# lRomul/sensorium

Hardware: AMD Instinct MI355X
Metric: training clips/sec/GPU (DwiseNeuro fwd+bwd, B=32 T=32 36x64) at 1/2/4/8 GPUs (higher is better)
Workload: dtype bf16

## Files before the change

### sensorium_amd/csrc/dwn_gemm.hip

```cpp
#include "dwn_internal.h"
#include "dwn_launch.h"
#include <type_traits>
int k_zero(void* p, size_t nbytes, hipStream_t s);

#ifndef NN_DMA_NST
#define NN_DMA_NST 3
#endif
#ifndef NN_F32_X3
#define NN_F32_X3 1
#endif

typedef __attribute__((ext_vector_type(8))) short bf16x8_t;
typedef __attribute__((ext_vector_type(4))) short s16x4_t;
typedef __attribute__((ext_vector_type(4))) float f32x4_t;

template <typename T> struct Mma;
template <> struct Mma<bf16_t> {
    static __device__ __forceinline__ void run(const uint4& a, const uint4& b, f32x4_t& acc) {
        acc = __builtin_amdgcn_mfma_f32_16x16x32_bf16(__builtin_bit_cast(bf16x8_t, a),
                                                      __builtin_bit_cast(bf16x8_t, b), acc, 0, 0, 0);
    }
};
template <> struct Mma<float> {
    static __device__ __forceinline__ void run(const uint4& a, const uint4& b, f32x4_t& acc) {
// ... 441 lines not shown
                if (CROWS >= 64 ? (wm == prow0 / 64 || CROWS == 128) : (wm == prow0 / 64)) {
#pragma unroll
                    for (int i = 0; i < 4; ++i) {
                        const int trow = wm * 64 + i * 16 + lr;
                        if (trow >= prow0 && trow < prow0 + CROWS) {
#pragma unroll
                            for (int j = 0; j < NJ; ++j) {
                                const int col = wn * (BN / 2) + j * 16 + lg * 4;
                                unsigned char* dst = sC + sc_off(trow - prow0, col * (int)sizeof(T));
                                if (EPI == EPI_STORE_CAT && n0 + col < g.N) {
                                    const float4 bv = *reinterpret_cast<const float4*>(g.bias + ccol0 + n0 + col);
                                    acc[i][j][0] += bv.x; acc[i][j][1] += bv.y; acc[i][j][2] += bv.z; acc[i][j][3] += bv.w;
                                }
                                if constexpr (TT<T>::IS_BF16) {
                                    uint2 v;
                                    v.x = pk_bf16(acc[i][j][0], acc[i][j][1]);
                                    v.y = pk_bf16(acc[i][j][2], acc[i][j][3]);
                                    *reinterpret_cast<uint2*>(dst) = v;
                                } else {
                                    *reinterpret_cast<float4*>(dst) =
                                        make_float4(acc[i][j][0], acc[i][j][1], acc[i][j][2], acc[i][j][3]);
                                }
                            }
                        }
                    }
                }
                bar();
                if constexpr (fast) {
#pragma unroll
                    for (int it = 0; it < CROWS * CPR / 256; ++it) {
                        const int row = tid / CPR + it * (256 / CPR);
                        const int m = mp + row;
                        const uint4 raw = *reinterpret_cast<const uint4*>(sC + sc_off(row, ch_e * 16));
                        float v[KC];
                        unpack16<T>(raw, v);
                        if constexpr (EPI == EPI_DH3) {
                            float y[KC], dh[KC];
                            unpack16<T>(zraw[it], y);
#pragma unroll
                            for (int i = 0; i < KC; ++i) dh[i] = fmaf(y[i], sc3[i], sh3[i]);
                            silu_grad_n<KC>(dh, dh);
#pragma unroll
                            for (int i = 0; i < KC; ++i) dh[i] = fmaf(v[i], gt3[i], gp3[i]) * dh[i];
                            const uint4 packed = pack16<T>(dh);
                            *reinterpret_cast<uint4*>(Cp + (i64)m * g.ldc + ccol0 + ncol_e) = packed;
                            if (g.stats) {
                                float r[KC];
                                unpack16<T>(packed, r);
#pragma unroll
                                for (int i = 0; i < KC; ++i) { st0[i] += r[i]; st1[i] = fmaf(r[i], y[i], st1[i]); }
                            }
                            continue;
                        }
                        *reinterpret_cast<uint4*>(Cp + (i64)m * g.ldc + ccol0 + ncol_e) = raw;
                        if (g.stats) {
#pragma unroll
                            for (int i = 0; i < KC; ++i) { st0[i] += v[i]; st1[i] += v[i] * v[i]; }
                        }
                        if constexpr (EPI == EPI_DG) {
                            float y[KC];
                            unpack16<T>(zraw[it], y);
#pragma unroll
                            for (int i = 0; i < KC; ++i) dgp[i] += v[i] * y[i];
                        }
                    }
                } else {
#pragma unroll
                for (int it = 0; it < CROWS * CPR / 256; ++it) {
                    const int row = tid / CPR + it * (256 / CPR);
                    const int m = mp + row;
                    if (m >= g.M || ncol >= g.N) continue;
                    const uint4 raw = *reinterpret_cast<const uint4*>(sC + sc_off(row, ch * 16));
                    float v[KC];
                    unpack16<T>(raw, v);
                    if constexpr (EPI == EPI_DH3) {
                        const int b = g.rows_per_sample >= CROWS ? pb3 + (m >= pbound3 ? 1 : 0) : m / g.rows_per_sample;
                        float y[KC], dh[KC];
                        unpack16<T>(zraw[it], y);
                        if (b != gb3) {
                            gb3 = b;
                            ld_coef<KC>(g.gate3 + (i64)b * g.dg_ld + ncol, gt3);
                            ld_coef<KC>(g.dps3 + (i64)b * g.dg_ld + ncol, gp3);
                        }
#pragma unroll
                        for (int i = 0; i < KC; ++i) dh[i] = fmaf(y[i], sc3[i], sh3[i]);
                        silu_grad_n<KC>(dh, dh);
#pragma unroll
                        for (int i = 0; i < KC; ++i) dh[i] = fmaf(v[i], gt3[i], gp3[i]) * dh[i];
                        const uint4 packed = pack16<T>(dh);
                        *reinterpret_cast<uint4*>(Cp + (i64)m * g.ldc + ccol0 + ncol) = packed;
                        if (g.stats) {
                            float r[KC];
                            unpack16<T>(packed, r);
#pragma unroll
                            for (int i = 0; i < KC; ++i) { st0[i] += r[i]; st1[i] = fmaf(r[i], y[i], st1[i]); }
                        }
                        continue;
                    }
                    *reinterpret_cast<uint4*>(Cp + (i64)m * g.ldc + ccol0 + ncol) = raw;
                    if (g.stats) {
#pragma unroll
                        for (int i = 0; i < KC; ++i) { st0[i] += v[i]; st1[i] += v[i] * v[i]; }
                    }
                    if constexpr (EPI == EPI_DG) {
                        const int b = m / g.rows_per_sample;
                        float y[KC];
                        unpack16<T>(zraw[it], y);
                        const int b_pass = mp / g.rows_per_sample;
                        if (b == b_pass) {
#pragma unroll
                            for (int i = 0; i < KC; ++i) dgp[i] += v[i] * y[i];
                        } else {
#pragma unroll
                            for (int i = 0; i < KC; ++i) atomicAdd(g.dg + (i64)b * g.dg_ld + ncol + i, v[i] * y[i]);
                        }
                    }
                }
                }
                if constexpr (EPI == EPI_DG) {
                    const int b_pass = mp / g.rows_per_sample;
                    dg_b = b_pass;
                    const int m_next = mp + CROWS;
                    const bool last = (pass == NPASS - 1) && (mt + 1 == mt_end);
                    const int b_next = (m_next < g.M ? m_next : g.M - 1) / g.rows_per_sample;
                    if (last || b_next != b_pass || m_next >= g.M) flush_dg();
                    else bar();
                } else {
                    bar();
                }
            }
        }
        if constexpr (single && HN) {
            if constexpr (EPI == EPI_READOUT) __syncthreads();
            store_a();
            __syncthreads();
        }
    };
    if constexpr (DMA) {
#pragma unroll
        for (int q = 0; q < NST - 1; ++q) dma_issue();
    }
    else if constexpr (!single) { load_a(mt_beg * BM, 0); load_b(0, mt_beg * BM); }
    for (int mt = mt_beg; mt < mt_end; ++mt) {
        const int m0_ = mt * BM;
        bool fast = m0_ + BM <= g.M;
        if constexpr (EPI == EPI_DG || EPI == EPI_DH3) fast = fast && (m0_ / g.rows_per_sample == (m0_ + BM - 1) / g.rows_per_sample);
        if constexpr (EPI == EPI_READOUT) fast = false;
        using T_ = std::true_type;
        using F_ = std::false_type;
        if constexpr (single) {
            if (mt + 1 < mt_end) { if (fast) tile(mt, T_{}, T_{}); else tile(mt, T_{}, F_{}); }
            else { if (fast) tile(mt, F_{}, T_{}); else tile(mt, F_{}, F_{}); }
        } else if constexpr (DMA) {
            if (fast) tile(mt, F_{}, T_{}); else tile(mt, F_{}, F_{});
        } else {
            tile(mt, F_{}, F_{});
        }
    }
    if constexpr (EPI != EPI_READOUT) {
        if (g.stats) {
            if constexpr (EPI == EPI_DH3) {
                float mu3[KC], is3[KC];
                ld_coef<KC>(g.coef3 + 2 * (i64)g.coef3_ld + ncol_e, mu3);
                ld_coef<KC>(g.coef3 + 3 * (i64)g.coef3_ld + ncol_e, is3);
#pragma unroll
                for (int i = 0; i < KC; ++i) st1[i] = is3[i] * fmaf(-mu3[i], st0[i], st1[i]);
            }
            if (tid < 2 * BN) lred[tid] = 0.f;
            __syncthreads();
            DET_WAVES_BEGIN
            if (ncol < g.N) {
#pragma unroll
                for (int i = 0; i < KC; ++i) {
                    atomicAdd(&lred[ch * KC + i], st0[i]);
                    atomicAdd(&lred[BN + ch * KC + i], st1[i]);
                }
            }
            DET_WAVES_END
            __syncthreads();
            DET_ENTER();
            if (tid < 2 * BN) {
                int col = tid % BN, which = tid / BN;
                if (n0 + col < g.N)
                    stat_add(g.stats, (int)(blockIdx.x % DWN_NREP), g.stat_nchan, which, ccol0 + n0 + col, lred[tid]);
            }
        }
    }
    DET_EXIT();
}

template <typename T, int ALD, int EPI, int BNv, int SINGLE>
static int launch_nn_k(const GemmNN& g, hipStream_t s) {
    const int BM = 128;
    const int ntm = (g.M + BM - 1) / BM;
    const int ntn = (g.N + BNv - 1) / BNv;
    const int bpc = resident_bpc(gemm_nn_kernel<T, ALD, EPI, BNv, SINGLE>, 256, 0, 1);
    int nranges = (256 * bpc) / (ntn * g.groups);
    if (nranges > ntm) nranges = ntm;
    if (nranges < 1) nranges = 1;
    while (nranges > 1 && (nranges * ntn) % 8 != 0) --nranges;
    if ((nranges * ntn) % 8 != 0) nranges = 8;
    dim3 grid(nranges * ntn, g.groups);
    if constexpr (!TT<T>::IS_BF16 && NN_F32_X3 != 0) {
        if (g.f32_split != 0) {
            hipLaunchKernelGGL((gemm_nn_kernel<T, ALD, EPI, BNv, SINGLE, true>), grid, dim3(256), 0, s, g);
            DWN_CHECK_LAUNCH();
            return 0;
        }
    }
    hipLaunchKernelGGL((gemm_nn_kernel<T, ALD, EPI, BNv, SINGLE>), grid, dim3(256), 0, s, g);
    DWN_CHECK_LAUNCH();
    return 0;
}

template <int ALD, int EPI> struct HasSingle {
    static constexpr bool value = (ALD == LD_PLAIN && (EPI == EPI_STORE || EPI == EPI_DG || EPI == EPI_DH3)) || (ALD == LD_PE && EPI == EPI_STORE);
};
template <int ALD, int EPI> struct HasSingle2 {
    static constexpr bool value = ALD == LD_PLAIN && (EPI == EPI_STORE || EPI == EPI_DG || EPI == EPI_DH3);
};

static bool nn_use_dma(const GemmNN& g, int bn) {
    if (g.K % 64 != 0 || g.K < 128 || (g.epi == EPI_STORE_CAT && g.K1 % 64 != 0)) return false;
    if (g.epi == EPI_READOUT) return false;
    if (g.b_sample_stride) return true;
    const long long tiles = (long long)((g.M + 127) / 128) * ((g.N + bn - 1) / bn) * g.groups;
    return tiles <= 5 * 256 && g.K >= 512;
}

template <typename T, int ALD, int EPI>
static int launch_nn_t(const GemmNN& g, hipStream_t s) {
    constexpr int BK = 128 / (int)sizeof(T);
    const bool n64 = g.N <= 64 || (EPI == EPI_DH3 && !(TT<T>::IS_BF16 && g.N % 128 == 0));
    if constexpr (HasSingle<ALD, EPI>::value) {
        if (g.K <= BK) return n64 ? launch_nn_k<T, ALD, EPI, 64, 1>(g, s) : launch_nn_k<T, ALD, EPI, 128, 1>(g, s);
    }
    if constexpr (HasSingle2<ALD, EPI>::value) {
        if (g.K <= 2 * BK && !g.b_sample_stride)
            return n64 ? launch_nn_k<T, ALD, EPI, 64, 2>(g, s) : launch_nn_k<T, ALD, EPI, 128, 2>(g, s);
    }
    if constexpr (ALD == LD_PLAIN && TT<T>::IS_BF16) {
        if (nn_use_dma(g, n64 ? 64 : 128))
            return n64 ? launch_nn_k<T, ALD, EPI, 64, 3>(g, s) : launch_nn_k<T, ALD, EPI, 128, 3>(g, s);
    }
    return n64 ? launch_nn_k<T, ALD, EPI, 64, 0>(g, s) : launch_nn_k<T, ALD, EPI, 128, 0>(g, s);
}

template <typename T>
static int launch_nn_d(const GemmNN& g, hipStream_t s) {
    if (g.K % TT<T>::KC != 0) return dwn_set_error(-2, "gemm_nn: K must be a multiple of the 16-byte vector");
    if (g.epi == EPI_READOUT) {
        if (g.a_kind == LD_BNACT) return launch_nn_t<T, LD_BNACT, EPI_READOUT>(g, s);
        if (g.a_kind == LD_PLAIN) return launch_nn_t<T, LD_PLAIN, EPI_READOUT>(g, s);
        return dwn_set_error(-3, "gemm_nn: unsupported loader for readout epilogue");
    }
    if (g.N % TT<T>::KC != 0) return dwn_set_error(-2, "gemm_nn: N must be a multiple of the 16-byte vector");
    if (g.epi == EPI_DG) {
        if (g.s3 || g.t3) return dwn_set_error(-3, "gemm_nn: the dg epilogue reads the activated z3; s3/t3 must be NULL");
        if (g.a_kind == LD_PLAIN && g.groups == 1) return launch_nn_t<T, LD_PLAIN, EPI_DG>(g, s);
        return dwn_set_error(-3, "gemm_nn: unsupported loader for dg epilogue");
    }
    if (g.epi == EPI_DH3) {
        if (g.a_kind != LD_PLAIN || g.groups != 1 || !g.y3 || !g.gate3 || !g.dps3 || !g.coef3 || g.rows_per_sample <= 0)
            return dwn_set_error(-3, "gemm_nn: the dh3 epilogue needs a plain loader, groups == 1, y3, gate3, dps3, coef3, rows_per_sample");
        return launch_nn_t<T, LD_PLAIN, EPI_DH3>(g, s);
    }
    if (g.epi == EPI_STORE_CAT) {
        if (g.a_kind != LD_PLAIN || g.groups != 1 || g.K1 <= 0 || g.K1 % TT<T>::KC || !g.a2 || !g.bias)
            return dwn_set_error(-3, "gemm_nn: K-concat epilogue needs a plain loader, groups == 1, a2, bias and K1 % vector == 0");
        return launch_nn_t<T, LD_PLAIN, EPI_STORE_CAT>(g, s);
    }
    switch (g.a_kind) {
        case LD_PLAIN: return launch_nn_t<T, LD_PLAIN, EPI_STORE>(g, s);
        case LD_PE: return launch_nn_t<T, LD_PE, EPI_STORE>(g, s);
        case LD_BNACT: return launch_nn_t<T, LD_BNACT, EPI_STORE>(g, s);
        case LD_AFFINE2: return launch_nn_t<T, LD_AFFINE2, EPI_STORE>(g, s);
        case LD_GATE: return launch_nn_t<T, LD_GATE, EPI_STORE>(g, s);
    }
    return dwn_set_error(-3, "gemm_nn: unsupported loader kind");
}

int launch_gemm_nn(const GemmNN& g, int dtype, hipStream_t s) {
    if (g.M <= 0 || g.N <= 0 || g.K <= 0) return 0;
    if (g.b_sample_stride) {
        const int bk = dtype == DWN_BF16 ? 64 : 32;
        if (g.b_rows_per_sample <= 0 || g.b_rows_per_sample % 128 || g.groups != 1 || g.K <= bk)
            return dwn_set_error(-2, "gemm_nn: per-sample weights need b_rows_per_sample % 128 == 0, groups == 1, K > one k-tile");
    }
    if (gemm_nn_kd_eligible(g, dtype)) return launch_gemm_nn_kd(g, s);
    if (gemm_nn_xl_eligible(g, dtype)) return launch_gemm_nn_xl(g, s);
    return dtype == DWN_BF16 ? launch_nn_d<bf16_t>(g, s) : launch_nn_d<float>(g, s);
}

#ifndef TN_MINW_PLAIN
#define TN_MINW_PLAIN 3
#endif
template <typename T> static __device__ __forceinline__ uint4 ones_vec();
template <> __device__ __forceinline__ uint4 ones_vec<bf16_t>() { return make_uint4(0x3F803F80u, 0x3F803F80u, 0x3F803F80u, 0x3F803F80u); }
template <> __device__ __forceinline__ uint4 ones_vec<float>() { return make_uint4(0x3F800000u, 0x3F800000u, 0x3F800000u, 0x3F800000u); }
template <typename T> struct TnCfg;
template <> struct TnCfg<bf16_t> { static constexpr int PAD = 32; };
template <> struct TnCfg<float>  { static constexpr int PAD = 64; };

template <int PLD, int QLD> struct TnOcc {
    static constexpr int value = (PLD == LD_AFFINE2 || PLD == LD_DY3 || QLD == LD_AFFINE2 || QLD == LD_DY3) ? 2 : TN_MINW_PLAIN;
};
template <typename T, int PLD, int QLD>
__global__ __launch_bounds__(256, (TnOcc<PLD, QLD>::value)) void gemm_tn_kernel(const GemmTN g) {
    constexpr int KC = TT<T>::KC;
    constexpr int BR = 128, BC = 128, BMK = TT<T>::IS_BF16 ? 64 : 32;
    constexpr int RS = BR * (int)sizeof(T) + TnCfg<T>::PAD;
    constexpr int CPR = BR / KC;
    constexpr int NCH = BMK * CPR / 256;
    __shared__ __attribute__((aligned(16))) unsigned char smem[2 * BMK * RS];
    unsigned char* sP = smem;
    unsigned char* sQ = smem + BMK * RS;

    const int tid = threadIdx.x;
    const int ntc = (g.Cc + BC - 1) / BC;
    int tile_id = blockIdx.x, split_id = blockIdx.y;
    {
        const unsigned total = gridDim.x * gridDim.y, bid = blockIdx.x + gridDim.x * blockIdx.y;
        if ((total & 7u) == 0u) {
            const unsigned lid = (bid & 7u) * (total >> 3) + (bid >> 3);
            tile_id = (int)(lid % gridDim.x);
            split_id = (int)(lid / gridDim.x);
        }
    }
    const int rt = tile_id / ntc, ct = tile_id % ntc;
    const int r0 = rt * BR, c0 = ct * BC;
    const int grp = blockIdx.z;
    const int Rl = g.R_load > 0 ? g.R_load : g.R;
    const int pcol0 = grp * Rl, qcol0 = grp * g.Cc;
    i64 mbeg = (i64)split_id * g.rows_per_split;
    i64 mend = mbeg + g.rows_per_split;
    if (mend > g.M) mend = g.M;
    i64 dw_off = 0;
    if (g.rows_per_sample > 0) {
        const int b = split_id / g.splits_per_sample, j = split_id % g.splits_per_sample;
        mbeg = (i64)b * g.rows_per_sample + (i64)j * g.rows_per_split;
        mend = mbeg + g.rows_per_split;
        const i64 send = (i64)(b + 1) * g.rows_per_sample;
        if (mend > send) mend = send;
        dw_off = (i64)b * g.dw_sample_stride;
    }

    const int wave = tid >> 6, lane = tid & 63;
    const int wm = wave >> 1, wn = wave & 1;
    const int lr = lane & 15, lg = lane >> 4;

    f32x4_t acc[4][4];
#pragma unroll
    for (int i = 0; i < 4; ++i)
#pragma unroll
        for (int j = 0; j < 4; ++j) acc[i][j] = f32x4_t{0.f, 0.f, 0.f, 0.f};

    uint4 p1[NCH], p2[NCH], q1[NCH], q2[NCH];
    i64 ld_mb = 0;
    const int chq = tid % CPR;
    const int rcol = r0 + chq * KC, ccol = c0 + chq * KC;
    const bool rok = rcol < Rl, cok = ccol < g.Cc;
    ColCoef<(PLD == LD_PE || PLD == LD_CAT1) ? LD_PLAIN : PLD, T> cfp;
    ColCoef<QLD == LD_PE ? LD_PLAIN : QLD, T> cfq;
    if (rok) cfp.load(g.p, pcol0 + rcol);
    if (cok) cfq.load(g.q, qcol0 + ccol);
    const T* Pp = reinterpret_cast<const T*>(g.p.p);
    const T* Pq = reinterpret_cast<const T*>(g.p.q);
    const T* Qp = reinterpret_cast<const T*>(g.q.p);
    const T* Qq = reinterpret_cast<const T*>(g.q.q);
    i64 pld = g.p.ld;
    int pcol = pcol0 + rcol;
    [[maybe_unused]] bool p_ones = false;
    if constexpr (PLD == LD_CAT1) {
        if (rcol >= g.p.cat_c1 + g.p.cat_c2) p_ones = true;
        else if (rcol >= g.p.cat_c1) { Pp = Pq; pld = g.p.ld2; pcol = rcol - g.p.cat_c1; }
    }
    auto load_tiles = [&](i64 mb) {
        ld_mb = mb;
#pragma unroll
        for (int i = 0; i < NCH; ++i) {
            i64 m = mb + tid / CPR + (256 / CPR) * i;
            const bool mok = m < mend;
            i64 offp = (mok && rok) ? m * pld + pcol : 0;
            if constexpr (PLD == LD_CAT1) { if (p_ones) offp = 0; }
            const i64 offq = (mok && cok) ? m * g.q.ld + qcol0 + ccol : 0;
            if constexpr (PLD != LD_PE) {
                p1[i] = *reinterpret_cast<const uint4*>(Pp + offp);
                if constexpr (decltype(cfp)::two_tensors) p2[i] = *reinterpret_cast<const uint4*>(Pq + offp);
            } else {
                p1[i] = (mok && rok) ? load_op_packed<LD_PE, T>(g.p, m, pcol0 + rcol) : make_uint4(0, 0, 0, 0);
            }
            if constexpr (QLD != LD_PE) {
                q1[i] = *reinterpret_cast<const uint4*>(Qp + offq);
                if constexpr (decltype(cfq)::two_tensors) q2[i] = *reinterpret_cast<const uint4*>(Qq + offq);
            } else {
                q1[i] = (mok && cok) ? load_op_packed<LD_PE, T>(g.q, m, qcol0 + ccol) : make_uint4(0, 0, 0, 0);
            }
        }
    };
    auto store_tiles = [&]() {
        const uint4 z4 = make_uint4(0, 0, 0, 0);
#pragma unroll
        for (int i = 0; i < NCH; ++i) {
            int mrow = tid / CPR + (256 / CPR) * i;
            const i64 m = ld_mb + mrow;
            const bool mok = m < mend;
            uint4 vp, vq;
            if constexpr (PLD == LD_PE) vp = p1[i];
            else if constexpr (PLD == LD_CAT1) vp = !(mok && rok) ? z4 : p_ones ? ones_vec<T>() : p1[i];
            else if constexpr (decltype(cfp)::two_tensors) vp = (mok && rok) ? cfp.apply(g.p, (unsigned)m, p1[i], p2[i]) : z4;
            else vp = (mok && rok) ? cfp.apply(g.p, (unsigned)m, p1[i], z4) : z4;
            if constexpr (QLD == LD_PE) vq = q1[i];
            else if constexpr (decltype(cfq)::two_tensors) vq = (mok && cok) ? cfq.apply(g.q, (unsigned)m, q1[i], q2[i]) : z4;
            else vq = (mok && cok) ? cfq.apply(g.q, (unsigned)m, q1[i], z4) : z4;
            *reinterpret_cast<uint4*>(sP + mrow * RS + chq * 16) = vp;
            *reinterpret_cast<uint4*>(sQ + mrow * RS + chq * 16) = vq;
        }
    };

    if (mbeg < mend) {
        load_tiles(mbeg);
        store_tiles();
    }
    __syncthreads();
    for (i64 mb = mbeg; mb < mend; mb += BMK) {
        const bool has_next = (mb + BMK) < mend;
        if (has_next) load_tiles(mb + BMK);
        if constexpr (TT<T>::IS_BF16) {
            const int q = lr >> 2, p = lr & 3;
#pragma unroll
            for (int kb = 0; kb < BMK / 32; ++kb) {
                bf16x8_t af[4], bfr[4];
                const int rb = kb * 32 + 8 * lg + q;
#pragma unroll
                for (int i = 0; i < 4; ++i) {
                    int colb = (wm * 64 + i * 16 + 4 * p) * 2;
                    auto lo = __builtin_amdgcn_ds_read_tr16_b64_v4i16(
                        (__attribute__((address_space(3))) s16x4_t*)(sP + rb * RS + colb));
                    auto hi = __builtin_amdgcn_ds_read_tr16_b64_v4i16(
                        (__attribute__((address_space(3))) s16x4_t*)(sP + (rb + 4) * RS + colb));
                    af[i] = bf16x8_t{lo[0], lo[1], lo[2], lo[3], hi[0], hi[1], hi[2], hi[3]};
                }
#pragma unroll
                for (int j = 0; j < 4; ++j) {
                    int colb = (wn * 64 + j * 16 + 4 * p) * 2;
                    auto lo = __builtin_amdgcn_ds_read_tr16_b64_v4i16(
                        (__attribute__((address_space(3))) s16x4_t*)(sQ + rb * RS + colb));
                    auto hi = __builtin_amdgcn_ds_read_tr16_b64_v4i16(
                        (__attribute__((address_space(3))) s16x4_t*)(sQ + (rb + 4) * RS + colb));
                    bfr[j] = bf16x8_t{lo[0], lo[1], lo[2], lo[3], hi[0], hi[1], hi[2], hi[3]};
                }
#pragma unroll
                for (int i = 0; i < 4; ++i)
#pragma unroll
                    for (int j = 0; j < 4; ++j)
                        acc[i][j] = __builtin_amdgcn_mfma_f32_16x16x32_bf16(af[i], bfr[j], acc[i][j], 0, 0, 0);
            }
        } else {
#pragma unroll
            for (int ks = 0; ks < BMK / 4; ++ks) {
                float af[4], bfr[4];
#pragma unroll
                for (int i = 0; i < 4; ++i)
                    af[i] = *reinterpret_cast<const float*>(sP + (ks * 4 + lg) * RS + (wm * 64 + i * 16 + lr) * 4);
#pragma unroll
                for (int j = 0; j < 4; ++j)
                    bfr[j] = *reinterpret_cast<const float*>(sQ + (ks * 4 + lg) * RS + (wn * 64 + j * 16 + lr) * 4);
#pragma unroll
                for (int i = 0; i < 4; ++i)
#pragma unroll
                    for (int j = 0; j < 4; ++j)
                        acc[i][j] = __builtin_amdgcn_mfma_f32_16x16x4f32(af[i], bfr[j], acc[i][j], 0, 0, 0);
            }
        }
        __syncthreads();
        if (has_next) {
            store_tiles();
            __syncthreads();
        }
    }
    if (mbeg >= mend) { DET_EXIT(); return; }
    DET_ENTER();
    float* dw = g.dw + (i64)grp * g.R * g.lddw + dw_off;
#pragma unroll
    for (int i = 0; i < 4; ++i)
#pragma unroll
        for (int j = 0; j < 4; ++j)
#pragma unroll
            for (int r = 0; r < 4; ++r) {
                int rr = r0 + wm * 64 + i * 16 + lg * 4 + r;
                int cc = c0 + wn * 64 + j * 16 + lr;
                if (rr < g.R && cc < g.Cc) {
                    if (g.overwrite == 2) dw[(i64)rr * g.lddw + cc] = acc[i][j][r];
                    else if (g.dw_f64) atomicAdd(reinterpret_cast<double*>(g.dw) + (i64)grp * g.R * g.lddw + dw_off + (i64)rr * g.lddw + cc, (double)acc[i][j][r]);
                    else atomicAdd(dw + (i64)rr * g.lddw + cc, acc[i][j][r]);
                }
            }
    DET_EXIT();
}

#define TRY_(x) do { int rc__ = (x); if (rc__ != 0) return rc__; } while (0)
#ifndef TN_SLOTS
#define TN_SLOTS 2
#endif
#ifndef TN_F64_SLOTS
#define TN_F64_SLOTS 2
#endif
template <typename T, int PLD, int QLD>
static int launch_tn_t(const GemmTN& g_in, hipStream_t s) {
    GemmTN g = g_in;
    if (g.rows_per_sample > 0) {
        if (g.groups != 1 || g.M % g.rows_per_sample) return dwn_set_error(-2, "gemm_tn: per-sample mode needs groups == 1 and M % rows_per_sample == 0");
        int bpc = resident_bpc(gemm_tn_kernel<T, PLD, QLD>, 256, 0, 1);
        const int nb = g.M / g.rows_per_sample;
        const int tiles = ((g.R + 127) / 128) * ((g.Cc + 127) / 128);
        if (bpc > TN_SLOTS) bpc = TN_SLOTS;
        int J = (256 * bpc) / (tiles * nb);
        const int maxj = (g.rows_per_sample + 511) / 512;
        if (J > maxj) J = maxj;
        if (J < 1) J = 1;
        int rows = (g.rows_per_sample + J - 1) / J;
        rows = (rows + 63) / 64 * 64;
        g.rows_per_split = rows;
        g.splits_per_sample = (g.rows_per_sample + rows - 1) / rows;
        g.nsplit = nb * g.splits_per_sample;
    } else if (g.nsplit <= 0) {
        int bpc = resident_bpc(gemm_tn_kernel<T, PLD, QLD>, 256, 0, 1);
        if (bpc > TN_SLOTS) bpc = TN_SLOTS;
        if (g.dw_f64 && bpc > TN_F64_SLOTS) bpc = TN_F64_SLOTS;
        const int tiles = ((g.R + 127) / 128) * ((g.Cc + 127) / 128) * g.groups;
        int want = (256 * bpc) / tiles;
        const int maxsplit = (int)((g.M + 511) / 512);
        if (want > maxsplit) want = maxsplit;
        if (want < 1) want = 1;
        const int tiles_g = ((g.R + 127) / 128) * ((g.Cc + 127) / 128);
        for (int w = want; w >= 1 && w > want - 8; --w) {
            i64 rows = (g.M + w - 1) / w;
            rows = (rows + 63) / 64 * 64;
            g.rows_per_split = (int)rows;
            g.nsplit = (int)((g.M + rows - 1) / rows);
            if (((tiles_g * g.nsplit) & 7) == 0) break;
        }
        if (((tiles_g * g.nsplit) & 7) != 0) {
            i64 rows = (g.M + want - 1) / want;
            rows = (rows + 63) / 64 * 64;
            g.rows_per_split = (int)rows;
            g.nsplit = (int)((g.M + rows - 1) / rows);
        }
    }
    if (g.dw_f64 && (g.overwrite || g.rows_per_sample > 0)) return dwn_set_error(-2, "gemm_tn: dw_f64 excludes overwrite and per-sample mode");
    if (g.overwrite) {
        if (g.rows_per_sample > 0 || g.lddw != g.Cc) return dwn_set_error(-2, "gemm_tn: overwrite needs lddw == Cc and no per-sample mode");
        if (g.nsplit == 1) g.overwrite = 2;
        else TRY_(k_zero(g.dw, (size_t)g.groups * g.R * g.lddw * sizeof(float), s));
    }
    dim3 grid(((g.R + 127) / 128) * ((g.Cc + 127) / 128), g.nsplit, g.groups);
    hipLaunchKernelGGL((gemm_tn_kernel<T, PLD, QLD>), grid, dim3(256), 0, s, g);
    DWN_CHECK_LAUNCH();
    return 0;
}

template <typename T>
static int launch_tn_d(const GemmTN& g, hipStream_t s) {
    const int Rl = g.R_load > 0 ? g.R_load : g.R;
    if (Rl % TT<T>::KC != 0 || g.Cc % TT<T>::KC != 0)
        return dwn_set_error(-2, "gemm_tn: R and Cc must be multiples of the 16-byte vector");
    const int pk = g.p_kind, qk = g.q_kind;
    if (pk == LD_AFFINE2 && qk == LD_PE) return launch_tn_t<T, LD_AFFINE2, LD_PE>(g, s);
    if (pk == LD_PLAIN && qk == LD_BNACT) return launch_tn_t<T, LD_PLAIN, LD_BNACT>(g, s);
    if (pk == LD_PLAIN && qk == LD_GATE) return launch_tn_t<T, LD_PLAIN, LD_GATE>(g, s);
    if (pk == LD_PLAIN && qk == LD_PLAIN) return launch_tn_t<T, LD_PLAIN, LD_PLAIN>(g, s);
    if (pk == LD_AFFINE2 && qk == LD_PLAIN) return launch_tn_t<T, LD_AFFINE2, LD_PLAIN>(g, s);
    if (pk == LD_CAT1 && qk == LD_PLAIN) {
        if (g.p.cat_c1 <= 0 || g.p.cat_c2 < 0 || g.p.cat_c1 % TT<T>::KC || g.p.cat_c2 % TT<T>::KC || g.groups != 1 ||
            g.R < g.p.cat_c1 + g.p.cat_c2 || (g.p.cat_c2 > 0 && !g.p.q))
            return dwn_set_error(-2, "gemm_tn: LD_CAT1 needs groups == 1, segment widths in 16-byte vectors and R >= cat_c1 + cat_c2");
        return launch_tn_t<T, LD_CAT1, LD_PLAIN>(g, s);
    }
    return dwn_set_error(-3, "gemm_tn: unsupported loader combination");
}

int launch_gemm_tn(const GemmTN& g_in, int dtype, hipStream_t s) {
    if (g_in.M <= 0 || g_in.R <= 0 || g_in.Cc <= 0) return 0;
    const GemmTN& g = g_in;
    return dtype == DWN_BF16 ? launch_tn_d<bf16_t>(g, s) : launch_tn_d<float>(g, s);
}

static __device__ __forceinline__ unsigned pwb_pack2(float a, float b) { return pk_bf16(a, b); }
namespace pwb {
constexpr int CIN = 64, BM = 128;
constexpr int RS = 160;
template <int NKC> struct Cfg {
    static constexpr int E = NKC * 64, KCAT = E + CIN;
    static constexpr int WRS = KCAT * 2 + 16;
    static constexpr int SW_BYTES = CIN * WRS, SD_BYTES = BM * RS, SX_BYTES = BM * RS;
    static constexpr int MAP_INTS = 512;
    static constexpr int LDS_BYTES = SW_BYTES + 2 * SD_BYTES + 2 * SX_BYTES + 7 * CIN * 4 + MAP_INTS * 4;
};
}
struct PwbGather { const int* hinv; const int* winv; int Hin, Win, Hout, Wout; };
template <int NKC>
__global__ __launch_bounds__(512) __attribute__((amdgpu_waves_per_eu(2, 2))) void pw_bwd_fused_kernel(const bf16_t* __restrict__ dh1, const bf16_t* __restrict__ a0,
                                                       const bf16_t* __restrict__ bp, const float* __restrict__ r3,
                                                       bf16_t* __restrict__ da0, float* __restrict__ tacc, int M,
                                                       const bf16_t* __restrict__ res, const float* __restrict__ res_coef, int res_n,
                                                       const PwbGather gq) {
    using namespace pwb;
    constexpr int E = Cfg<NKC>::E, KCAT = Cfg<NKC>::KCAT, WRS = Cfg<NKC>::WRS;
    constexpr int SW_BYTES = Cfg<NKC>::SW_BYTES, SD_BYTES = Cfg<NKC>::SD_BYTES, SX_BYTES = Cfg<NKC>::SX_BYTES;
    extern __shared__ __attribute__((aligned(16))) unsigned char pwb_smem[];
    unsigned char* const smem = pwb_smem;
    unsigned char* sW = smem;
    unsigned char* sD = smem + SW_BYTES;
    unsigned char* sX = sD + 2 * SD_BYTES;
    float* sR3 = reinterpret_cast<float*>(sX + 2 * SX_BYTES);
    const int tid = threadIdx.x, wave = tid >> 6, lane = tid & 63;
    const int lr = lane & 15, lg = lane >> 4;
    const int wm = wave & 3, wn = wave >> 2;
    if (tid < CIN) sR3[tid] = r3[tid];
    const bool gather = res && gq.hinv;
    if (res) for (int i = tid; i < (gather ? 3 : 1) * res_n * CIN; i += 512) sR3[CIN + i] = res_coef[i];
    int* sMap = reinterpret_cast<int*>(sR3 + 7 * CIN);
    if (gather) for (int i = tid; i < gq.Hin + gq.Win; i += 512) sMap[i] = i < gq.Hin ? gq.hinv[i] : gq.winv[i - gq.Hin];
    const RasterIdx ridx(gather ? gq.Hin : 1, gather ? gq.Win : 1);
    for (int c = tid; c < CIN * (KCAT / 8); c += 512) {
        const int n = c / (KCAT / 8), kc8 = c % (KCAT / 8);
        *reinterpret_cast<uint4*>(sW + n * WRS + kc8 * 16) = *reinterpret_cast<const uint4*>(bp + (size_t)n * KCAT + kc8 * 8);
    }
    f32x4_t acc_dw[NKC][2], acc_ga[2], acc_s[2];
#pragma unroll
    for (int k = 0; k < NKC; ++k) { acc_dw[k][0] = f32x4_t{0, 0, 0, 0}; acc_dw[k][1] = f32x4_t{0, 0, 0, 0}; }
    acc_ga[0] = acc_ga[1] = acc_s[0] = acc_s[1] = f32x4_t{0, 0, 0, 0};
    const int ntiles = M / BM;
    const int ch = tid & 7;
    const int row_a = tid >> 3;
    struct Pair { uint4 lo, hi; };
    Pair rd[NKC], rx;
    auto fetch_a0 = [&](int tile) {
        const bf16_t* src = a0 + ((size_t)tile * BM + row_a) * CIN + ch * 8;
        return Pair{*reinterpret_cast<const uint4*>(src), *reinterpret_cast<const uint4*>(src + (size_t)64 * CIN)};
    };
    auto fetch_chunk = [&](int tile, int kc) {
        const bf16_t* src = dh1 + ((size_t)tile * BM + row_a) * E + kc * 64 + ch * 8;
        return Pair{*reinterpret_cast<const uint4*>(src), *reinterpret_cast<const uint4*>(src + (size_t)64 * E)};
    };
    int tile = blockIdx.x;
    {
        const int t0 = tile < ntiles ? tile : 0;
        rx = fetch_a0(t0);
#pragma unroll
        for (int kc = 0; kc < NKC; ++kc) rd[kc] = fetch_chunk(t0, kc);
    }
    __syncthreads();
    const int q = lr >> 2, p = lr & 3;
    const bf16x8_t ones = {(short)0x3F80, (short)0x3F80, (short)0x3F80, (short)0x3F80, (short)0x3F80, (short)0x3F80, (short)0x3F80, (short)0x3F80};
    int tpar = 0, step = 0;
    for (; tile < ntiles; tile += gridDim.x, tpar ^= 1) {
        const size_t m0 = (size_t)tile * BM;
        const int ntile = tile + (int)gridDim.x < ntiles ? tile + (int)gridDim.x : tile;
        unsigned char* sXt = sX + tpar * SX_BYTES;
        *reinterpret_cast<uint4*>(sXt + row_a * RS + ch * 16) = rx.lo;
        *reinterpret_cast<uint4*>(sXt + (row_a + 64) * RS + ch * 16) = rx.hi;
        rx = fetch_a0(ntile);
        f32x4_t acc_da[2][2];
        uint2 rres[2][2][2];
        bool rgat[2] = {true, true};
#pragma unroll
        for (int i = 0; i < 2; ++i) { acc_da[i][0] = f32x4_t{0, 0, 0, 0}; acc_da[i][1] = f32x4_t{0, 0, 0, 0}; }
#pragma unroll
        for (int kc = 0; kc < NKC; ++kc) {
            unsigned char* sDk = sD + ((step + kc) & 1) * SD_BYTES;
            *reinterpret_cast<uint4*>(sDk + row_a * RS + ch * 16) = rd[kc].lo;
            *reinterpret_cast<uint4*>(sDk + (row_a + 64) * RS + ch * 16) = rd[kc].hi;
            nn_lds_barrier();
            rd[kc] = fetch_chunk(ntile, kc);
            if (kc == NKC - 3 && res) {
#pragma unroll
                for (int i = 0; i < 2; ++i) {
                    size_t rrow = m0 + wm * 32 + i * 16 + lr;
                    if (gather) {
                        unsigned bt; int hi, wi;
                        ridx.decode((unsigned)rrow, bt, hi, wi);
                        const int ho = sMap[hi], wo = sMap[gq.Hin + wi];
                        rgat[i] = ho >= 0 && wo >= 0;
                        rrow = rgat[i] ? ((size_t)bt * gq.Hout + ho) * gq.Wout + wo : 0;
                    }
#pragma unroll
                    for (int j = 0; j < 2; ++j) {
                        const bf16_t* rp_ = res + rrow * (size_t)(res_n * CIN) + wn * 32 + j * 16 + 4 * lg;
                        rres[i][j][0] = *reinterpret_cast<const uint2*>(rp_);
                        rres[i][j][1] = *reinterpret_cast<const uint2*>(rp_ + (res_n > 1 ? CIN : 0));
                    }
                }
            }
#pragma unroll
            for (int kb = 0; kb < 2; ++kb) {
                bf16x8_t af[2], wf[2];
#pragma unroll
                for (int i = 0; i < 2; ++i)
                    af[i] = *reinterpret_cast<const bf16x8_t*>(sDk + (wm * 32 + i * 16 + lr) * RS + (kb * 4 + lg) * 16);
#pragma unroll
                for (int j = 0; j < 2; ++j)
                    wf[j] = *reinterpret_cast<const bf16x8_t*>(sW + (wn * 32 + j * 16 + lr) * WRS + (kc * 64 + kb * 32 + lg * 8) * 2);
#pragma unroll
                for (int i = 0; i < 2; ++i)
#pragma unroll
                    for (int j = 0; j < 2; ++j)
                        acc_da[i][j] = __builtin_amdgcn_mfma_f32_16x16x32_bf16(wf[j], af[i], acc_da[i][j], 0, 0, 0);
            }
#pragma unroll
            for (int kb = 0; kb < BM / 32; ++kb) {
                const int rb = kb * 32 + 8 * lg + q;
                bf16x8_t ef, cf[2];
                {
                    const int colb = (wm * 16 + 4 * p) * 2;
                    auto lo = __builtin_amdgcn_ds_read_tr16_b64_v4i16((__attribute__((address_space(3))) s16x4_t*)(sDk + rb * RS + colb));
                    auto hi = __builtin_amdgcn_ds_read_tr16_b64_v4i16((__attribute__((address_space(3))) s16x4_t*)(sDk + (rb + 4) * RS + colb));
                    ef = bf16x8_t{lo[0], lo[1], lo[2], lo[3], hi[0], hi[1], hi[2], hi[3]};
                }
#pragma unroll
                for (int j = 0; j < 2; ++j) {
                    const int colb = (wn * 32 + j * 16 + 4 * p) * 2;
                    auto lo = __builtin_amdgcn_ds_read_tr16_b64_v4i16((__attribute__((address_space(3))) s16x4_t*)(sXt + rb * RS + colb));
                    auto hi = __builtin_amdgcn_ds_read_tr16_b64_v4i16((__attribute__((address_space(3))) s16x4_t*)(sXt + (rb + 4) * RS + colb));
                    cf[j] = bf16x8_t{lo[0], lo[1], lo[2], lo[3], hi[0], hi[1], hi[2], hi[3]};
                }
#pragma unroll
                for (int j = 0; j < 2; ++j)
                    acc_dw[kc][j] = __builtin_amdgcn_mfma_f32_16x16x32_bf16(ef, cf[j], acc_dw[kc][j], 0, 0, 0);
            }
            if (kc == 0) {
#pragma unroll
                for (int kb = 0; kb < 2; ++kb) {
                    bf16x8_t af[2], wf[2];
#pragma unroll
                    for (int i = 0; i < 2; ++i)
                        af[i] = *reinterpret_cast<const bf16x8_t*>(sXt + (wm * 32 + i * 16 + lr) * RS + (kb * 4 + lg) * 16);
#pragma unroll
                    for (int j = 0; j < 2; ++j)
                        wf[j] = *reinterpret_cast<const bf16x8_t*>(sW + (wn * 32 + j * 16 + lr) * WRS + (E + kb * 32 + lg * 8) * 2);
#pragma unroll
                    for (int i = 0; i < 2; ++i)
#pragma unroll
                        for (int j = 0; j < 2; ++j)
                            acc_da[i][j] = __builtin_amdgcn_mfma_f32_16x16x32_bf16(wf[j], af[i], acc_da[i][j], 0, 0, 0);
                }
#pragma unroll
                for (int kb = 0; kb < BM / 32; ++kb) {
                    const int rb = kb * 32 + 8 * lg + q;
                    bf16x8_t ef, cf[2];
                    {
                        const int colb = (wm * 16 + 4 * p) * 2;
                        auto lo = __builtin_amdgcn_ds_read_tr16_b64_v4i16((__attribute__((address_space(3))) s16x4_t*)(sXt + rb * RS + colb));
                        auto hi = __builtin_amdgcn_ds_read_tr16_b64_v4i16((__attribute__((address_space(3))) s16x4_t*)(sXt + (rb + 4) * RS + colb));
                        ef = bf16x8_t{lo[0], lo[1], lo[2], lo[3], hi[0], hi[1], hi[2], hi[3]};
                    }
#pragma unroll
                    for (int j = 0; j < 2; ++j) {
                        const int colb = (wn * 32 + j * 16 + 4 * p) * 2;
                        auto lo = __builtin_amdgcn_ds_read_tr16_b64_v4i16((__attribute__((address_space(3))) s16x4_t*)(sXt + rb * RS + colb));
                        auto hi = __builtin_amdgcn_ds_read_tr16_b64_v4i16((__attribute__((address_space(3))) s16x4_t*)(sXt + (rb + 4) * RS + colb));
                        cf[j] = bf16x8_t{lo[0], lo[1], lo[2], lo[3], hi[0], hi[1], hi[2], hi[3]};
                    }
#pragma unroll
                    for (int j = 0; j < 2; ++j) {
                        acc_ga[j] = __builtin_amdgcn_mfma_f32_16x16x32_bf16(ef, cf[j], acc_ga[j], 0, 0, 0);
                        if (wm == 0) acc_s[j] = __builtin_amdgcn_mfma_f32_16x16x32_bf16(ones, cf[j], acc_s[j], 0, 0, 0);
                    }
                }
            }
        }
        step += NKC;
#pragma unroll
        for (int i = 0; i < 2; ++i)
#pragma unroll
            for (int j = 0; j < 2; ++j) {
                const size_t m = m0 + wm * 32 + i * 16 + lr;
                const int n = wn * 32 + j * 16 + 4 * lg;
                const float4 b4 = *reinterpret_cast<const float4*>(sR3 + n);
                float o[4] = {acc_da[i][j][0] + b4.x, acc_da[i][j][1] + b4.y, acc_da[i][j][2] + b4.z, acc_da[i][j][3] + b4.w};
                if (res) {
                    const int rc = res_n * CIN;
                    float x4[4] = {0.f, 0.f, 0.f, 0.f};
                    if (gather) {
                        const uint2 xv = *reinterpret_cast<const uint2*>(sXt + (wm * 32 + i * 16 + lr) * RS + n * 2);
                        x4[0] = __uint_as_float(xv.x << 16); x4[1] = __uint_as_float(xv.x & 0xffff0000u);
                        x4[2] = __uint_as_float(xv.y << 16); x4[3] = __uint_as_float(xv.y & 0xffff0000u);
                    }
#pragma unroll
                    for (int jj = 0; jj < 2; ++jj) {
                        if (jj >= res_n || !rgat[i]) break;
                        const uint2 rv = rres[i][j][jj];
                        const float4 c4 = *reinterpret_cast<const float4*>(sR3 + CIN + jj * CIN + n);
                        float t[4] = {c4.x * __uint_as_float(rv.x << 16), c4.y * __uint_as_float(rv.x & 0xffff0000u),
                                      c4.z * __uint_as_float(rv.y << 16), c4.w * __uint_as_float(rv.y & 0xffff0000u)};
                        if (gather) {
                            const float4 a2 = *reinterpret_cast<const float4*>(sR3 + CIN + rc + jj * CIN + n);
                            const float4 a3 = *reinterpret_cast<const float4*>(sR3 + CIN + 2 * rc + jj * CIN + n);
                            t[0] += fmaf(a2.x, x4[0], a3.x); t[1] += fmaf(a2.y, x4[1], a3.y);
                            t[2] += fmaf(a2.z, x4[2], a3.z); t[3] += fmaf(a2.w, x4[3], a3.w);
                        }
                        o[0] += t[0]; o[1] += t[1]; o[2] += t[2]; o[3] += t[3];
                    }
                }
                uint2 v = make_uint2(pwb_pack2(o[0], o[1]), pwb_pack2(o[2], o[3]));
                *reinterpret_cast<uint2*>(da0 + m * CIN + n) = v;
            }
    }
    DET_ENTER();
#pragma unroll
    for (int kc = 0; kc < NKC; ++kc)
#pragma unroll
        for (int j = 0; j < 2; ++j)
#pragma unroll
            for (int r = 0; r < 4; ++r)
                atomicAdd(tacc + (size_t)(kc * 64 + wm * 16 + 4 * lg + r) * CIN + wn * 32 + j * 16 + lr, acc_dw[kc][j][r]);
#pragma unroll
    for (int j = 0; j < 2; ++j) {
#pragma unroll
        for (int r = 0; r < 4; ++r)
            atomicAdd(tacc + (size_t)(E + wm * 16 + 4 * lg + r) * CIN + wn * 32 + j * 16 + lr, acc_ga[j][r]);
        if (wm == 0 && lg == 0) atomicAdd(tacc + (size_t)KCAT * CIN + wn * 32 + j * 16 + lr, acc_s[j][0]);
    }
    DET_EXIT();
}


bool pw_bwd_fused_supported(int dtype, long long M, int E, int Cin) {
    return dtype == DWN_BF16 && (E == 448 || E == 384) && Cin == pwb::CIN && M > 0 && M % pwb::BM == 0 && M <= 0x7fffffffLL;
}
template <int NKC>
static int launch_pw_bwd_fused_t(const void* dh1, const void* a0, const void* bp, const float* r3, void* da0, float* tacc,
                                 long long M, const void* res, const float* res_coef, int res_n, const PwbGather& gq, hipStream_t s) {
    auto kern = pw_bwd_fused_kernel<NKC>;
    {
        hipError_t e = lds_opt_in(kern, pwb::Cfg<NKC>::LDS_BYTES);
        if (e != hipSuccess) return dwn_set_error((int)e, hipGetErrorString(e));
    }
    int grid = 256;
    if (grid > (int)(M / pwb::BM)) grid = (int)(M / pwb::BM);
    hipLaunchKernelGGL(kern, dim3(grid), dim3(512), pwb::Cfg<NKC>::LDS_BYTES, s, (const bf16_t*)dh1, (const bf16_t*)a0,
                       (const bf16_t*)bp, r3, (bf16_t*)da0, tacc, (int)M, (const bf16_t*)res, res_coef, res_n, gq);
    DWN_CHECK_LAUNCH();
    return 0;
}
int launch_pw_bwd_fused(const void* dh1, const void* a0, const void* bp, const float* r3, void* da0, float* tacc,
                        long long M, int E, int Cin, int dtype, const void* res, const float* res_coef, int res_n,
                        const int* hinv, const int* winv, int Hin, int Win, int Hout, int Wout, hipStream_t s) {
    PwbGather gq; gq.hinv = hinv; gq.winv = winv; gq.Hin = Hin; gq.Win = Win; gq.Hout = Hout; gq.Wout = Wout;
    if (res && hinv && (!winv || Hin <= 0 || Win <= 0 || Hout <= 0 || Wout <= 0 || M % ((long long)Hin * Win) || Hin + Win > 512))
        return dwn_set_error(-2, "pw_bwd_fused: the gathered shortcut form needs both inverse maps, M = frames * Hin * Win and Hin + Win <= 512");
    if (!pw_bwd_fused_supported(dtype, M, E, Cin))
        return dwn_set_error(-3, "pw_bwd_fused: built for bf16, Cin = 64, E = 448 or 384, M % 128 == 0 only");
    if (res && (!res_coef || res_n < 1 || res_n > 2)) return dwn_set_error(-3, "pw_bwd_fused: the residual term needs res_coef and res_n in {1, 2}");
    return E == 448 ? launch_pw_bwd_fused_t<7>(dh1, a0, bp, r3, da0, tacc, M, res, res_coef, res_n, gq, s)
                    : launch_pw_bwd_fused_t<6>(dh1, a0, bp, r3, da0, tacc, M, res, res_coef, res_n, gq, s);
}
```

Measured before the change: 1475.

## Add register-ring prefetch with double-buffered LDS and fold ones-row bias into TN GEMM

For plain and concat-with-ones weight-gradient GEMMs, the kernel now keeps a register ring of prefetched global tiles and ping-pongs two LDS buffers, so each k-step needs one barrier instead of two. For the concat-with-ones case it accumulates column sums of Q in registers and writes them to the bias rows from the last real row tile. This removes the extra 128-row tile that existed only to hold the ones row. The cost is more registers and twice the shared memory, with occupancy capped at 2 for these variants. Ablation macros and an optional LDS-staged flush are also added but are off by default.

```diff
diff --git a/sensorium_amd/csrc/dwn_gemm.hip b/sensorium_amd/csrc/dwn_gemm.hip
--- a/sensorium_amd/csrc/dwn_gemm.hip
+++ b/sensorium_amd/csrc/dwn_gemm.hip
@@ -767,17 +767,35 @@
 template <> struct TnCfg<bf16_t> { static constexpr int PAD = 32; };
 template <> struct TnCfg<float>  { static constexpr int PAD = 64; };
 
+#ifndef TN_RING
+#define TN_RING 2
+#endif
+#ifndef TN_FLUSH_LDS
+#define TN_FLUSH_LDS 0
+#endif
+#ifndef TN_ONES_FOLD
+#define TN_ONES_FOLD 1
+#endif
+template <int PLD, int QLD> struct TnRing {
+    static constexpr int value = ((PLD == LD_PLAIN || PLD == LD_CAT1) && QLD == LD_PLAIN) ? TN_RING : 0;
+};
 template <int PLD, int QLD> struct TnOcc {
-    static constexpr int value = (PLD == LD_AFFINE2 || PLD == LD_DY3 || QLD == LD_AFFINE2 || QLD == LD_DY3) ? 2 : TN_MINW_PLAIN;
+    static constexpr int value = (TnRing<PLD, QLD>::value > 0 || PLD == LD_AFFINE2 || PLD == LD_DY3 || QLD == LD_AFFINE2 || QLD == LD_DY3)
+                                     ? 2 : TN_MINW_PLAIN;
 };
+#if defined(TN_ABL_LOADONLY) && !defined(TN_ABL_NOFLUSH)
+#define TN_ABL_NOFLUSH
+#endif
 template <typename T, int PLD, int QLD>
-__global__ __launch_bounds__(256, (TnOcc<PLD, QLD>::value)) void gemm_tn_kernel(const GemmTN g) {
+__global__ __launch_bounds__(256, (TnOcc<PLD, QLD>::value)) void gemm_tn_kernel(const GemmTN g, const int ones_rt, const int ones_n) {
     constexpr int KC = TT<T>::KC;
     constexpr int BR = 128, BC = 128, BMK = TT<T>::IS_BF16 ? 64 : 32;
     constexpr int RS = BR * (int)sizeof(T) + TnCfg<T>::PAD;
     constexpr int CPR = BR / KC;
     constexpr int NCH = BMK * CPR / 256;
-    __shared__ __attribute__((aligned(16))) unsigned char smem[2 * BMK * RS];
+    constexpr int RING = TnRing<PLD, QLD>::value;
+    constexpr int TILE = 2 * BMK * RS;
+    __shared__ __attribute__((aligned(16))) unsigned char smem[(RING > 0 ? 2 : 1) * TILE];
     unsigned char* sP = smem;
     unsigned char* sQ = smem + BMK * RS;
 
@@ -878,11 +896,157 @@
             if constexpr (QLD == LD_PE) vq = q1[i];
             else if constexpr (decltype(cfq)::two_tensors) vq = (mok && cok) ? cfq.apply(g.q, (unsigned)m, q1[i], q2[i]) : z4;
             else vq = (mok && cok) ? cfq.apply(g.q, (unsigned)m, q1[i], z4) : z4;
+#ifdef TN_ABL_LOADONLY
+            asm volatile("" :: "v"(vp.x), "v"(vp.y), "v"(vp.z), "v"(vp.w), "v"(vq.x), "v"(vq.y), "v"(vq.z), "v"(vq.w));
+#else
             *reinterpret_cast<uint4*>(sP + mrow * RS + chq * 16) = vp;
             *reinterpret_cast<uint4*>(sQ + mrow * RS + chq * 16) = vq;
+#endif
         }
     };
 
+    auto mma_tile = [&](const unsigned char* tP, const unsigned char* tQ) __attribute__((always_inline)) {
+#ifdef TN_ABL_LOADONLY
+        (void)tP; (void)tQ;
+#else
+        if constexpr (TT<T>::IS_BF16) {
+            const int q = lr >> 2, p = lr & 3;
+#pragma unroll
+            for (int kb = 0; kb < BMK / 32; ++kb) {
+                bf16x8_t af[4], bfr[4];
+                const int rb = kb * 32 + 8 * lg + q;
+#pragma unroll
+                for (int i = 0; i < 4; ++i) {
+                    int colb = (wm * 64 + i * 16 + 4 * p) * 2;
+                    auto lo = __builtin_amdgcn_ds_read_tr16_b64_v4i16(
+                        (__attribute__((address_space(3))) s16x4_t*)(tP + rb * RS + colb));
+                    auto hi = __builtin_amdgcn_ds_read_tr16_b64_v4i16(
+                        (__attribute__((address_space(3))) s16x4_t*)(tP + (rb + 4) * RS + colb));
+                    af[i] = bf16x8_t{lo[0], lo[1], lo[2], lo[3], hi[0], hi[1], hi[2], hi[3]};
+                }
+#pragma unroll
+                for (int j = 0; j < 4; ++j) {
+                    int colb = (wn * 64 + j * 16 + 4 * p) * 2;
+                    auto lo = __builtin_amdgcn_ds_read_tr16_b64_v4i16(
+                        (__attribute__((address_space(3))) s16x4_t*)(tQ + rb * RS + colb));
+                    auto hi = __builtin_amdgcn_ds_read_tr16_b64_v4i16(
+                        (__attribute__((address_space(3))) s16x4_t*)(tQ + (rb + 4) * RS + colb));
+                    bfr[j] = bf16x8_t{lo[0], lo[1], lo[2], lo[3], hi[0], hi[1], hi[2], hi[3]};
+                }
+#pragma unroll
+                for (int i = 0; i < 4; ++i)
+#pragma unroll
+                    for (int j = 0; j < 4; ++j)
+                        acc[i][j] = __builtin_amdgcn_mfma_f32_16x16x32_bf16(af[i], bfr[j], acc[i][j], 0, 0, 0);
+            }
+        } else {
+#pragma unroll
+            for (int ks = 0; ks < BMK / 4; ++ks) {
+                float af[4], bfr[4];
+#pragma unroll
+                for (int i = 0; i < 4; ++i)
+                    af[i] = *reinterpret_cast<const float*>(tP + (ks * 4 + lg) * RS + (wm * 64 + i * 16 + lr) * 4);
+#pragma unroll
+                for (int j = 0; j < 4; ++j)
+                    bfr[j] = *reinterpret_cast<const float*>(tQ + (ks * 4 + lg) * RS + (wn * 64 + j * 16 + lr) * 4);
+#pragma unroll
+                for (int i = 0; i < 4; ++i)
+#pragma unroll
+                    for (int j = 0; j < 4; ++j)
+                        acc[i][j] = __builtin_amdgcn_mfma_f32_16x16x4f32(af[i], bfr[j], acc[i][j], 0, 0, 0);
+            }
+        }
+#endif
+    };
+    if constexpr (RING > 0) {
+        constexpr int U = (RING % 2 == 0) ? RING : 2 * RING;
+        uint4 rp[RING][NCH], rq[RING][NCH];
+        [[maybe_unused]] const bool sum_q = PLD == LD_CAT1 && rt == ones_rt;
+        [[maybe_unused]] f32x4_t cs0 = {0.f, 0.f, 0.f, 0.f}, cs1 = {0.f, 0.f, 0.f, 0.f};
+        auto ring_load = [&](uint4 (&dp)[NCH], uint4 (&dq)[NCH], i64 mb) __attribute__((always_inline)) {
+#pragma unroll
+            for (int i = 0; i < NCH; ++i) {
+                const i64 m = mb + tid / CPR + (256 / CPR) * i;
+                const bool mok = m < mend;
+                i64 offp = (mok && rok) ? m * pld + pcol : 0;
+                if constexpr (PLD == LD_CAT1) { if (p_ones) offp = 0; }
+                const i64 offq = (mok && cok) ? m * g.q.ld + qcol0 + ccol : 0;
+                dp[i] = *reinterpret_cast<const uint4*>(Pp + offp);
+                dq[i] = *reinterpret_cast<const uint4*>(Qp + offq);
+            }
+        };
+        auto ring_store = [&](const uint4 (&dp)[NCH], const uint4 (&dq)[NCH], i64 mb, int buf) __attribute__((always_inline)) {
+#pragma unroll
+            for (int i = 0; i < NCH; ++i) {
+                const int mrow = tid / CPR + (256 / CPR) * i;
+                const bool mok = mb + mrow < mend;
+                const bool pk = mok && rok, qk = mok && cok;
+                uint4 vp = make_uint4(dp[i].x, dp[i].y, dp[i].z, dp[i].w);
+                if constexpr (PLD == LD_CAT1) { if (p_ones) vp = ones_vec<T>(); }
+                vp = make_uint4(pk ? vp.x : 0u, pk ? vp.y : 0u, pk ? vp.z : 0u, pk ? vp.w : 0u);
+                const uint4 vq = make_uint4(qk ? dq[i].x : 0u, qk ? dq[i].y : 0u, qk ? dq[i].z : 0u, qk ? dq[i].w : 0u);
+                if constexpr (PLD == LD_CAT1) {
+                    if constexpr (TT<T>::IS_BF16) {
+                        cs0 += f32x4_t{__uint_as_float(vq.x << 16), __uint_as_float(vq.x & 0xffff0000u),
+                                       __uint_as_float(vq.y << 16), __uint_as_float(vq.y & 0xffff0000u)};
+                        cs1 += f32x4_t{__uint_as_float(vq.z << 16), __uint_as_float(vq.z & 0xffff0000u),
+                                       __uint_as_float(vq.w << 16), __uint_as_float(vq.w & 0xffff0000u)};
+                    } else {
+                        cs0 += f32x4_t{__uint_as_float(vq.x), __uint_as_float(vq.y), __uint_as_float(vq.z), __uint_as_float(vq.w)};
+                    }
+                }
+#ifdef TN_ABL_LOADONLY
+                asm volatile("" :: "v"(vp.x), "v"(vp.y), "v"(vp.z), "v"(vp.w), "v"(vq.x), "v"(vq.y), "v"(vq.z), "v"(vq.w));
+#else
+                *reinterpret_cast<uint4*>(smem + buf * TILE + mrow * RS + chq * 16) = vp;
+                *reinterpret_cast<uint4*>(smem + buf * TILE + BMK * RS + mrow * RS + chq * 16) = vq;
+#endif
+            }
+        };
+        if (mbeg < mend) {
+            const i64 nst = (mend - mbeg + BMK - 1) / BMK;
+#pragma unroll
+            for (int k = 0; k < RING; ++k) ring_load(rp[k], rq[k], mbeg + (i64)k * BMK);
+            ring_store(rp[0], rq[0], mbeg, 0);
+            ring_load(rp[0], rq[0], mbeg + (i64)RING * BMK);
+            __syncthreads();
+            for (i64 t0 = 0; t0 < nst; t0 += U) {
+#pragma unroll
+                for (int u = 0; u < U; ++u) {
+                    const i64 t = t0 + u;
+                    if (t >= nst) break;
+                    ring_store(rp[(u + 1) % RING], rq[(u + 1) % RING], mbeg + (t + 1) * BMK, (u + 1) & 1);
+                    ring_load(rp[(u + 1) % RING], rq[(u + 1) % RING], mbeg + (t + 1 + RING) * BMK);
+                    mma_tile(smem + (u & 1) * TILE, smem + (u & 1) * TILE + BMK * RS);
+                    __syncthreads();
+                }
+            }
+#ifndef TN_ABL_NOFLUSH
+            if constexpr (PLD == LD_CAT1) {
+                if (sum_q) {
+                    float* red = reinterpret_cast<float*>(smem);
+                    float* mine = red + (tid / CPR) * BC + chq * KC;
+                    mine[0] = cs0[0]; mine[1] = cs0[1]; mine[2] = cs0[2]; mine[3] = cs0[3];
+                    if constexpr (KC == 8) { mine[4] = cs1[0]; mine[5] = cs1[1]; mine[6] = cs1[2]; mine[7] = cs1[3]; }
+                    __syncthreads();
+                    DET_ENTER();
+                    if (tid < BC && c0 + tid < g.Cc) {
+                        float sum = 0.f;
+#pragma unroll
+                        for (int r = 0; r < 256 / CPR; ++r) sum += red[r * BC + tid];
+                        for (int j = 0; j < ones_n; ++j) {
+                            const i64 at = dw_off + (i64)(g.R + j) * g.lddw + c0 + tid;
+                            if (g.overwrite == 2) g.dw[at] = sum;
+                            else if (g.dw_f64) atomicAdd(reinterpret_cast<double*>(g.dw) + at, (double)sum);
+                            else atomicAdd(g.dw + at, sum);
+                        }
+                    }
+                    __syncthreads();
+                }
+            }
+#endif
+        }
+    } else {
     if (mbeg < mend) {
         load_tiles(mbeg);
         store_tiles();
@@ -891,62 +1055,48 @@
     for (i64 mb = mbeg; mb < mend; mb += BMK) {
         const bool has_next = (mb + BMK) < mend;
         if (has_next) load_tiles(mb + BMK);
-        if constexpr (TT<T>::IS_BF16) {
-            const int q = lr >> 2, p = lr & 3;
-#pragma unroll
-            for (int kb = 0; kb < BMK / 32; ++kb) {
-                bf16x8_t af[4], bfr[4];
-                const int rb = kb * 32 + 8 * lg + q;
-#pragma unroll
-                for (int i = 0; i < 4; ++i) {
-                    int colb = (wm * 64 + i * 16 + 4 * p) * 2;
-                    auto lo = __builtin_amdgcn_ds_read_tr16_b64_v4i16(
-                        (__attribute__((address_space(3))) s16x4_t*)(sP + rb * RS + colb));
-                    auto hi = __builtin_amdgcn_ds_read_tr16_b64_v4i16(
-                        (__attribute__((address_space(3))) s16x4_t*)(sP + (rb + 4) * RS + colb));
-                    af[i] = bf16x8_t{lo[0], lo[1], lo[2], lo[3], hi[0], hi[1], hi[2], hi[3]};
-                }
-#pragma unroll
-                for (int j = 0; j < 4; ++j) {
-                    int colb = (wn * 64 + j * 16 + 4 * p) * 2;
-                    auto lo = __builtin_amdgcn_ds_read_tr16_b64_v4i16(
-                        (__attribute__((address_space(3))) s16x4_t*)(sQ + rb * RS + colb));
-                    auto hi = __builtin_amdgcn_ds_read_tr16_b64_v4i16(
-                        (__attribute__((address_space(3))) s16x4_t*)(sQ + (rb + 4) * RS + colb));
-                    bfr[j] = bf16x8_t{lo[0], lo[1], lo[2], lo[3], hi[0], hi[1], hi[2], hi[3]};
-                }
-#pragma unroll
-                for (int i = 0; i < 4; ++i)
-#pragma unroll
-                    for (int j = 0; j < 4; ++j)
-                        acc[i][j] = __builtin_amdgcn_mfma_f32_16x16x32_bf16(af[i], bfr[j], acc[i][j], 0, 0, 0);
-            }
-        } else {
-#pragma unroll
-            for (int ks = 0; ks < BMK / 4; ++ks) {
-                float af[4], bfr[4];
-#pragma unroll
-                for (int i = 0; i < 4; ++i)
-                    af[i] = *reinterpret_cast<const float*>(sP + (ks * 4 + lg) * RS + (wm * 64 + i * 16 + lr) * 4);
-#pragma unroll
-                for (int j = 0; j < 4; ++j)
-                    bfr[j] = *reinterpret_cast<const float*>(sQ + (ks * 4 + lg) * RS + (wn * 64 + j * 16 + lr) * 4);
-#pragma unroll
-                for (int i = 0; i < 4; ++i)
-#pragma unroll
-                    for (int j = 0; j < 4; ++j)
-                        acc[i][j] = __builtin_amdgcn_mfma_f32_16x16x4f32(af[i], bfr[j], acc[i][j], 0, 0, 0);
-            }
-        }
+        mma_tile(sP, sQ);
         __syncthreads();
         if (has_next) {
             store_tiles();
             __syncthreads();
         }
     }
+    }
     if (mbeg >= mend) { DET_EXIT(); return; }
+#ifdef TN_ABL_NOFLUSH
+#pragma unroll
+    for (int i = 0; i < 4; ++i)
+#pragma unroll
+        for (int j = 0; j < 4; ++j) asm volatile("" :: "v"(acc[i][j][0]), "v"(acc[i][j][1]), "v"(acc[i][j][2]), "v"(acc[i][j][3]));
+#else
     DET_ENTER();
     float* dw = g.dw + (i64)grp * g.R * g.lddw + dw_off;
+#if TN_FLUSH_LDS
+    if constexpr (RING > 0) {
+        if (g.overwrite != 2 && !g.dw_f64) {
+            constexpr int FS = 68;
+            static_assert(4 * 64 * FS * 4 <= 2 * TILE, "the flush staging must fit the tile buffers");
+            float* fq = reinterpret_cast<float*>(smem) + wave * 64 * FS;
+#pragma unroll
+            for (int i = 0; i < 4; ++i)
+#pragma unroll
+                for (int j = 0; j < 4; ++j)
+#pragma unroll
+                    for (int r = 0; r < 4; ++r) fq[(i * 16 + lg * 4 + r) * FS + j * 16 + lr] = acc[i][j][r];
+            __syncthreads();
+            const int cc = c0 + wn * 64 + lane;
+#pragma unroll 8
+            for (int rq_ = 0; rq_ < 64; ++rq_) {
+                const int rr = r0 + wm * 64 + rq_;
+                const float v = fq[rq_ * FS + lane];
+                if (rr < g.R && cc < g.Cc) atomicAdd(dw + (i64)rr * g.lddw + cc, v);
+            }
+            DET_EXIT();
+            return;
+        }
+    }
+#endif
 #pragma unroll
     for (int i = 0; i < 4; ++i)
 #pragma unroll
@@ -961,6 +1111,7 @@
                     else atomicAdd(dw + (i64)rr * g.lddw + cc, acc[i][j][r]);
                 }
             }
+#endif
     DET_EXIT();
 }
 
@@ -974,11 +1125,17 @@
 template <typename T, int PLD, int QLD>
 static int launch_tn_t(const GemmTN& g_in, hipStream_t s) {
     GemmTN g = g_in;
+    int ones_rt = -1, ones_n = 0;
+    if constexpr (PLD == LD_CAT1 && TnRing<PLD, QLD>::value > 0 && TN_ONES_FOLD != 0) {
+        const int cw = g.p.cat_c1 + g.p.cat_c2;
+        if (g.R > cw && cw % 128 == 0 && g.R_load <= 0) { ones_rt = cw / 128 - 1; ones_n = g.R - cw; }
+    }
+    const int Rm = g.R - ones_n;
     if (g.rows_per_sample > 0) {
         if (g.groups != 1 || g.M % g.rows_per_sample) return dwn_set_error(-2, "gemm_tn: per-sample mode needs groups == 1 and M % rows_per_sample == 0");
         int bpc = resident_bpc(gemm_tn_kernel<T, PLD, QLD>, 256, 0, 1);
         const int nb = g.M / g.rows_per_sample;
-        const int tiles = ((g.R + 127) / 128) * ((g.Cc + 127) / 128);
+        const int tiles = ((Rm + 127) / 128) * ((g.Cc + 127) / 128);
         if (bpc > TN_SLOTS) bpc = TN_SLOTS;
         int J = (256 * bpc) / (tiles * nb);
         const int maxj = (g.rows_per_sample + 511) / 512;
@@ -993,12 +1150,12 @@
         int bpc = resident_bpc(gemm_tn_kernel<T, PLD, QLD>, 256, 0, 1);
         if (bpc > TN_SLOTS) bpc = TN_SLOTS;
         if (g.dw_f64 && bpc > TN_F64_SLOTS) bpc = TN_F64_SLOTS;
-        const int tiles = ((g.R + 127) / 128) * ((g.Cc + 127) / 128) * g.groups;
+        const int tiles = ((Rm + 127) / 128) * ((g.Cc + 127) / 128) * g.groups;
         int want = (256 * bpc) / tiles;
         const int maxsplit = (int)((g.M + 511) / 512);
         if (want > maxsplit) want = maxsplit;
         if (want < 1) want = 1;
-        const int tiles_g = ((g.R + 127) / 128) * ((g.Cc + 127) / 128);
+        const int tiles_g = ((Rm + 127) / 128) * ((g.Cc + 127) / 128);
         for (int w = want; w >= 1 && w > want - 8; --w) {
             i64 rows = (g.M + w - 1) / w;
             rows = (rows + 63) / 64 * 64;
@@ -1019,8 +1176,9 @@
         if (g.nsplit == 1) g.overwrite = 2;
         else TRY_(k_zero(g.dw, (size_t)g.groups * g.R * g.lddw * sizeof(float), s));
     }
-    dim3 grid(((g.R + 127) / 128) * ((g.Cc + 127) / 128), g.nsplit, g.groups);
-    hipLaunchKernelGGL((gemm_tn_kernel<T, PLD, QLD>), grid, dim3(256), 0, s, g);
+    dim3 grid(((Rm + 127) / 128) * ((g.Cc + 127) / 128), g.nsplit, g.groups);
+    g.R = Rm;
+    hipLaunchKernelGGL((gemm_tn_kernel<T, PLD, QLD>), grid, dim3(256), 0, s, g, ones_rt, ones_n);
     DWN_CHECK_LAUNCH();
     return 0;
 }
```

Result: no change. 1466 (-0.6%).
